# david-cortes/poismf

Hardware: AMD Instinct MI355X
Metric: nonzeros/sec per full A+B sweep (higher is better)
Workload: dtype f32; 1 GPU; uniform 1000000x100000, 99949803 nnz (100000000 triplets, seed 1, duplicates summed), k=50, method=pg, maxupd=10, l2=1000, step=1e-09

## Files before the change

poismf_amd/csrc/poismf_hip.hip:

```cpp
#include <hip/hip_runtime.h>

#include <algorithm>
#include <atomic>
#include <cstdio>
#include <cstdlib>
#include <type_traits>

#include "plan.hpp"
#include "reg_eval.hpp"
#include "lane_eval.hpp"
#include "solvers.hpp"

#ifndef PMF_TU
#define PMF_TU -1
#endif
constexpr bool tu_has(int kmethod) { return PMF_TU == -1 || PMF_TU == kmethod; }

template <class EV, class = void> struct cold_constants : std::false_type {};
template <class EV> struct cold_constants<EV, std::void_t<decltype(EV::COLD_CONSTANTS)>> : std::integral_constant<bool, EV::COLD_CONSTANTS> {};

template <class EV, class T, int NC, int METHOD>
__device__ __forceinline__ void solve_row(const HalfArgs<T>& a, EV& ev, const T (&bs)[NC], unsigned lrow, unsigned nnz)
{
    const int k = a.geom.k;
    T* out = a.M + (size_t)(a.row_offset + lrow) * (size_t)k;
    T* out_p = a.Mp != nullptr ? a.Mp + (size_t)(a.row_offset + lrow) * (size_t)a.ldM : nullptr;
    T x[NC];
    if (nnz == 0) {
        T z = (T)0;
        asm volatile("" : "+v"(z));
        PMF_EW x[i] = z;
        ev.store_vec(out, x);
        if (out_p != nullptr) ev.store_vec(out_p, x);
        return;
    }
    ev.start_point(out, x);
    ev.n_eval = 0;

    T shift[NC];
    PMF_EW shift[i] = bs[i];
    const bool weighted = a.P.w != (T)1;
    if (weighted) {
        T cs[NC];
        PMF_EW cs[i] = (T)0;
        ev.tile_colsum(cs);
        T w_here = a.P.w;
        asm volatile("" : "+v"(w_here));
        const T wm1 = w_here - (T)1.;
        PMF_EW {
            shift[i] = cs[i] * wm1;
            shift[i] = shift[i] + bs[i];
        }
        if (METHOD == K_PG) {
            PMF_EW shift[i] = shift[i] * a.P.neg_step;
            if (a.P.neg_step2 != (T)1) { PMF_EW shift[i] = shift[i] * a.P.neg_step2; }
        }
    }

    SolveStats st;
    if constexpr (METHOD == K_EVAL) {
        T g[NC];
        double f;
        if (a.P.maxupd == 0) {
            f = (double)fun_single(ev, a.P, shift, x);
            grad_single(ev, a.P, shift, x, g, weighted);
        } else f = (double)fun_and_grad(ev, a.P, shift, x, g);
        ev.store_vec(out, g);
        if (out_p != nullptr) ev.store_vec(out_p, g);
        if (a.dec_rows != nullptr && ev.lane == 0 && ev.wid == 0 && ev.member == 0) {
            const unsigned long long fb = __builtin_bit_cast(unsigned long long, f);
            a.dec_rows[2 * (size_t)lrow] = (unsigned)fb;
            a.dec_rows[2 * (size_t)lrow + 1] = (unsigned)(fb >> 32);
        }
        return;
    } else if constexpr (METHOD == K_PG) {
        pg_row(ev, a.P, x, shift);
    } else if constexpr (METHOD == K_CG) {
        if constexpr (EV::MAY_CACHE) {
            if (a.P.limit_step && ev.pq_cap > 0 && nnz <= (unsigned)ev.pq_cap) cg_row_cached(ev, a.P, shift, x, weighted, st);
            else cg_row(ev, a.P, shift, x, weighted, st);
        } else cg_row(ev, a.P, shift, x, weighted, st);
    } else {
        T prev[NC];
        PMF_EW prev[i] = x[i];
        if (!a.reuse_prev) { PMF_EW x[i] = (T)1e-3; }
        (void)Tnc<T, NC, EV>::minimize(ev, a.P, shift, x, st);
        if (a.early_stop) {
            PMF_EW prev[i] = prev[i] - x[i];
            const T moved = ev.dot(prev, prev);
            if ((double)moved <= 1e-4 && ev.lane == 0 && ev.wid == 0 && ev.member == 0) atomicAdd(a.n_unchanged, 1u);
        }
    }
    ev.store_vec(out, x);
    if (out_p != nullptr) ev.store_vec(out_p, x);
#ifndef PMF_PROBE
    if (a.eval_rows != nullptr && ev.lane == 0 && ev.wid == 0 && ev.member == 0) a.eval_rows[lrow] += ev.n_eval;
#endif
    if (a.dec_rows != nullptr && ev.lane == 0 && ev.wid == 0 && ev.member == 0) {
        unsigned d0 = (unsigned)st.niter | ((unsigned)st.rc << 24), d1 = (unsigned)st.nfeval;
        if constexpr (cold_constants<EV>::value) asm volatile("" : "+v"(d0), "+v"(d1));
        a.dec_rows[2 * (size_t)lrow] = d0;
        a.dec_rows[2 * (size_t)lrow + 1] = d1;
    }
}

template <int METHOD, class T> __device__ __forceinline__ unsigned take_ticket(const HalfArgs<T>& a)
{
    unsigned st = 0u;
    if constexpr (METHOD != K_PG) {
        if (a.stop != nullptr) st = __hip_atomic_load(a.stop, __ATOMIC_RELAXED, __HIP_MEMORY_SCOPE_SYSTEM);
    }
    const unsigned t = atomicAdd(a.queue, 1u);
    return st != 0u ? 0xffffffffu : t;
}

template <class EV, class T, int NC, int METHOD, int NW>
__device__ __forceinline__ void sweep_rows(const HalfArgs<T>& a, EV& ev, unsigned char* smem)
{
    if (a.gate != nullptr && __hip_atomic_load(a.gate, __ATOMIC_RELAXED, __HIP_MEMORY_SCOPE_AGENT) == 0) return;
    ev.init(a.geom, a.F, smem);
    T bs[NC];
    ev.load_vec(a.bsum, bs);
    const RowDesc* desc = a.desc + a.perm_begin;
    if constexpr (EV::PIPELINED && (EV::PIPE_MW == 1 || (EV::PIPE_MW == 2 && METHOD == K_PG))) {
        unsigned r = blockIdx.x;
        auto ticket = [&]() -> unsigned {
            if (a.queue != nullptr) {
                if constexpr (NW > 1) {
                    unsigned* slot = ev.ticket_slot();
                    if (threadIdx.x == 0) *slot = take_ticket<METHOD>(a);
                    __syncthreads();
                    const unsigned t = uniform(*slot);
                    __syncthreads();
                    return t;
                }
                unsigned t = 0;
                if (ev.lane == 0) t = take_ticket<METHOD>(a);
                return uniform(t);
            }
            unsigned t = r;
            r += gridDim.x;
            if constexpr (METHOD != K_PG) {
                if (a.stop != nullptr && __hip_atomic_load(a.stop, __ATOMIC_RELAXED, __HIP_MEMORY_SCOPE_SYSTEM) != 0u) t = 0xffffffffu;
            }
            return t;
        };
        auto fetch = [&](unsigned t) -> RowDesc { return desc[t < a.nrows ? t : 0u]; };
        unsigned t0 = ticket(), t1 = ticket();
        RowDesc d0 = fetch(t0), d1 = fetch(t1);
        if (t0 < a.nrows) ev.fetch_meta(a.indices + (((unsigned long long)d0.p0_hi << 32) | d0.p0_lo), d0.nnz);
#ifdef PMF_PROBE
        unsigned probe_i = 0;
#endif
        while (t0 < a.nrows) {
            const unsigned long long p0 = ((unsigned long long)d0.p0_hi << 32) | d0.p0_lo;
            if (d0.nnz != 0) ev.gather(a.values + p0, d0.nnz);
            const unsigned t2 = ticket();
            const RowDesc d2 = fetch(t2);
            if (t1 < a.nrows) ev.fetch_meta(a.indices + (((unsigned long long)d1.p0_hi << 32) | d1.p0_lo), d1.nnz);
#ifdef PMF_PROBE
            ev.probe = (a.eval_rows != nullptr && blockIdx.x == 5 && threadIdx.x < WAVE && probe_i < 60) ? a.eval_rows + 16 * probe_i : nullptr;
            if (ev.probe != nullptr && ev.lane == 0) { ev.probe[10] = (unsigned)__builtin_amdgcn_s_memtime(); ev.probe[11] = d0.nnz; }
            probe_i++;
#endif
            solve_row<EV, T, NC, METHOD>(a, ev, bs, d0.lrow, d0.nnz);
            t0 = t1; d0 = d1;
            t1 = t2; d1 = d2;
        }
        return;
    } else {
        unsigned r = blockIdx.x;
        for (;;) {
            if (a.queue != nullptr) {
                if constexpr (NW > 1) {
                    unsigned* next_row = ev.ticket_slot();
                    if (threadIdx.x == 0) *next_row = take_ticket<METHOD>(a);
                    __syncthreads();
                    r = uniform(*next_row);
                    __syncthreads();
                } else {
                    unsigned t = 0;
                    if (ev.lane == 0) t = take_ticket<METHOD>(a);
                    r = uniform(t);
                }
            }
            if (r >= a.nrows) break;
            if constexpr (METHOD != K_PG) {
                if (a.queue == nullptr && a.stop != nullptr && uniform(__hip_atomic_load(a.stop, __ATOMIC_RELAXED, __HIP_MEMORY_SCOPE_SYSTEM)) != 0u) break;
            }
            const RowDesc d = desc[r];
            r += gridDim.x;
            const unsigned nnz = uniform(d.nnz);
            const unsigned long long p0 = ((unsigned long long)uniform(d.p0_hi) << 32) | uniform(d.p0_lo);
            if (nnz != 0) ev.begin_row(a.indices + p0, a.values + p0, nnz);
            solve_row<EV, T, NC, METHOD>(a, ev, bs, uniform(d.lrow), nnz);
        }
    }
}

template <class T, int NC, int METHOD, int SL, int NW>
__global__ __launch_bounds__(WAVE* NW) void half_sweep_kernel(const HalfArgs<T> a)
{
    extern __shared__ __attribute__((aligned(16))) unsigned char smem[];
    constexpr bool PF = SL > 0 && METHOD != K_TNCG;
    RowEval<T, NC, SL, NW, PF> ev;
    if constexpr (NW > 1) {
        if (a.arrive != nullptr && threadIdx.x == 0) atomicAdd(a.arrive, 1u);
    }
#ifdef PMF_TIMING
    const unsigned long long t_kernel = __builtin_amdgcn_s_memtime();
#endif
    sweep_rows<RowEval<T, NC, SL, NW, PF>, T, NC, METHOD, NW>(a, ev, smem);
#ifdef PMF_TIMING
    ev.tacc[5] = __builtin_amdgcn_s_memtime() - t_kernel;
    if (ev.lane == 0 && ev.wid == 0)
        for (int q = 0; q < 6; q++) atomicAdd(&g_pmf_timing[q], ev.tacc[q]);
#endif
}

template <class EV, class T, int NC, int METHOD>
__device__ __forceinline__ void team_rows(const HalfArgs<T>& a, EV& ev, unsigned char* smem)
{
    if (a.arrive != nullptr && threadIdx.x == 0) atomicAdd(a.arrive, 1u);
    ev.init(a.geom, a.F, smem);
    T bs[NC];
    ev.load_vec(a.bsum, bs);
    const RowDesc* desc = a.desc + a.perm_begin;
    const unsigned M = a.team_members;
    unsigned* box = ev.ticket_slot();
    if (threadIdx.x == 0) {
        const unsigned n = atomicAdd((unsigned*)a.team_buf, 1u);
        box[0] = n / M;
        box[1] = n % M;
    }
    __syncthreads();
    const unsigned team = uniform(box[0]);
    ev.member = (int)uniform(box[1]);
    __syncthreads();
    if ((size_t)(team + 1) * gt_team_words(M) + GT_HEAD_WORDS > GT_BUF_BYTES / 8) return;
    ev.tm_M = (int)M;
    ev.tm_seq = 0;
    ev.tm_words = a.team_buf + GT_HEAD_WORDS + (size_t)team * gt_team_words(M);
    ev.tm_err = a.team_err;
    ev.tm_spin = a.team_spin;
    unsigned long long* mail = ev.tm_words;
    constexpr unsigned END = 0xffffffffu;
    if (threadIdx.x == 0) atomicAdd((unsigned*)(mail + 2), 1u);
    if (a.team_spin <= 1u && threadIdx.x == 0) __hip_atomic_store(a.team_err, 1u, __ATOMIC_RELAXED, __HIP_MEMORY_SCOPE_AGENT);
    if (ev.wid == 0) {
        for (unsigned spins = 0;; spins++) {
            if (a.team_spin <= 1u) break;
            if (uniform((unsigned)gt_load(mail + 2)) >= M) break;
            if ((spins & 255u) == 255u) {
                if (uniform(__hip_atomic_load(a.team_err, __ATOMIC_RELAXED, __HIP_MEMORY_SCOPE_AGENT)) != 0) break;
                if (uniform(__hip_atomic_load(a.queue, __ATOMIC_RELAXED, __HIP_MEMORY_SCOPE_AGENT)) >= a.nrows) break;
            }
            if ((spins >> 6) > a.team_spin) { __hip_atomic_store(a.team_err, 1u, __ATOMIC_RELAXED, __HIP_MEMORY_SCOPE_AGENT); break; }
            __builtin_amdgcn_s_sleep(8);
        }
    }
    __syncthreads();
    for (unsigned rowno = 1;; rowno++) {
        if (ev.wid == 0) {
            unsigned tk = END;
            if (ev.member == 0) {
                unsigned t0 = 0;
                if (ev.lane == 0) t0 = take_ticket<METHOD>(a);
                tk = uniform(t0);
                if (tk >= a.nrows || uniform(__hip_atomic_load(a.team_err, __ATOMIC_RELAXED, __HIP_MEMORY_SCOPE_AGENT)) != 0) tk = END;
                gt_store(mail + (rowno & 1u), ((unsigned long long)rowno << 32) | tk);
            } else {
                unsigned seen = uniform(__hip_atomic_load(a.queue, __ATOMIC_RELAXED, __HIP_MEMORY_SCOPE_AGENT));
                for (unsigned spins = 0;; spins++) {
                    const unsigned long long v = gt_load(mail + (rowno & 1u));
                    const unsigned hi = uniform((unsigned)(v >> 32)), lo = uniform((unsigned)v);
                    if (hi == rowno) { tk = lo; break; }
                    if ((spins & 255u) == 255u) {
                        if (uniform(__hip_atomic_load(a.team_err, __ATOMIC_RELAXED, __HIP_MEMORY_SCOPE_AGENT)) != 0) break;
                        const unsigned q = uniform(__hip_atomic_load(a.queue, __ATOMIC_RELAXED, __HIP_MEMORY_SCOPE_AGENT));
                        if (q != seen) { seen = q; spins = 0; }
                        else if (rowno == 1u && q >= a.nrows) break;
                    }
                    if (spins > a.team_spin) { __hip_atomic_store(a.team_err, 1u, __ATOMIC_RELAXED, __HIP_MEMORY_SCOPE_AGENT); break; }
                    __builtin_amdgcn_s_sleep(4);
                }
            }
            box[0] = tk;
        }
        __syncthreads();
        const unsigned t = uniform(box[0]);
        __syncthreads();
        if (t >= a.nrows) break;
        const RowDesc d = desc[t];
        const unsigned nnz = uniform(d.nnz);
        const unsigned long long p0 = ((unsigned long long)uniform(d.p0_hi) << 32) | uniform(d.p0_lo);
        const unsigned S = ((nnz + M - 1u) / M + (EV::TEAM_ROUND - 1u)) / EV::TEAM_ROUND * EV::TEAM_ROUND;
        const unsigned off = (unsigned)ev.member * S;
        const unsigned mine = off < nnz ? (nnz - off < S ? nnz - off : S) : 0u;
        ev.begin_row(a.indices + p0 + (mine ? off : 0u), a.values + p0 + (mine ? off : 0u), mine);
        solve_row<EV, T, NC, METHOD>(a, ev, bs, uniform(d.lrow), nnz);
    }
}
template <class T, int NC, int METHOD, int SL, int NW>
__global__ __launch_bounds__(WAVE* NW) void half_sweep_giant_kernel(const HalfArgs<T> a)
{
    extern __shared__ __attribute__((aligned(16))) unsigned char smem[];
    constexpr bool PF = SL > 0 && METHOD != K_TNCG;
    using EV = RowEval<T, NC, SL, NW, PF, true>;
    EV ev;
// ... 542 lines not shown
```

poismf_amd/csrc/reg_eval.hpp:

```cpp
#pragma once
#include <type_traits>

#include "row_eval.hpp"

namespace pmf {

template <int I, int N, class Fn> __device__ __forceinline__ void static_for(Fn&& f)
{
    if constexpr (I < N) {
        f(std::integral_constant<int, I>{});
        static_for<I + 1, N>(f);
    }
}

template <int G, int U> __device__ __forceinline__ int group_bcast_i32(int v)
{
    return __builtin_amdgcn_ds_swizzle(v, (0x1f & ~(G - 1)) | (U << 5));
}
template <int G, int U> __device__ __forceinline__ unsigned group_bcast(unsigned v) { return (unsigned)group_bcast_i32<G, U>((int)v); }
template <int G, int U> __device__ __forceinline__ float group_bcast(float v)
{
    return __builtin_bit_cast(float, group_bcast_i32<G, U>(__builtin_bit_cast(int, v)));
}
template <int G, int U> __device__ __forceinline__ double group_bcast(double v)
{
    if constexpr (G == 16) return __builtin_amdgcn_update_dpp(0.0, v, 0x150 + U, 0xf, 0xf, true);
    const unsigned long long b = __builtin_bit_cast(unsigned long long, v);
    const unsigned lo = (unsigned)group_bcast_i32<G, U>((int)(unsigned)b);
    const unsigned hi = (unsigned)group_bcast_i32<G, U>((int)(unsigned)(b >> 32));
    return __builtin_bit_cast(double, ((unsigned long long)hi << 32) | lo);
}

template <int CTRL, class T> __device__ __forceinline__ T fold_pair(bool cls, T pa, T pb)
{
    const T own = cls ? pb : pa;
    const T send = cls ? pa : pb;
    return own + dpp_mov<CTRL>(send);
}
template <int CTRL, class T> __device__ __forceinline__ T fold_one(T pa) { return pa + dpp_mov<CTRL>(pa); }

template <int CTRL, int H, int NIN, class T> __device__ __forceinline__ void fold_level(bool cls, const T* in, T* out)
{
#pragma unroll
    for (int i = 0; i < H; i++) {
        if (i + H < NIN) out[i] = fold_pair<CTRL>(cls, in[i], in[i + H]);
        else if (i < NIN) out[i] = fold_one<CTRL>(in[i]);
        else out[i] = (T)0;
    }
}

__device__ __forceinline__ float coef_div(float num, float den)
{
    const float r = __builtin_amdgcn_rcpf(den);
    float q = num * r;
    const float e = __builtin_fmaf(-den, q, num);
    q = __builtin_fmaf(e, r, q);
    return __builtin_amdgcn_div_fixupf(q, den, num);
}
__device__ __forceinline__ double coef_div(double num, double den) { return num / den; }

#define PMF_FOLD2(CTRL, M0, M1, Q, A, B) \
    "v_add_f32_dpp " Q ", " A ", " A " " CTRL " row_mask:0xf bank_mask:" M0 "\n\t" \
    "v_add_f32_dpp " Q ", " B ", " B " " CTRL " row_mask:0xf bank_mask:" M1 "\n\t"
__device__ __forceinline__ void fold16_banked(const float (&p)[16], float (&q)[8])
{
    asm("s_nop 1\n\t"
        PMF_FOLD2("row_ror:8", "0x3", "0xc", "%0", "%8", "%16")
        PMF_FOLD2("row_ror:8", "0x3", "0xc", "%1", "%9", "%17")
        PMF_FOLD2("row_ror:8", "0x3", "0xc", "%2", "%10", "%18")
        PMF_FOLD2("row_ror:8", "0x3", "0xc", "%3", "%11", "%19")
        PMF_FOLD2("row_ror:8", "0x3", "0xc", "%4", "%12", "%20")
        PMF_FOLD2("row_ror:8", "0x3", "0xc", "%5", "%13", "%21")
        PMF_FOLD2("row_ror:8", "0x3", "0xc", "%6", "%14", "%22")
        PMF_FOLD2("row_ror:8", "0x3", "0xc", "%7", "%15", "%23")
        : "=&v"(q[0]), "=&v"(q[1]), "=&v"(q[2]), "=&v"(q[3]), "=&v"(q[4]), "=&v"(q[5]), "=&v"(q[6]), "=&v"(q[7])
        : "v"(p[0]), "v"(p[1]), "v"(p[2]), "v"(p[3]), "v"(p[4]), "v"(p[5]), "v"(p[6]), "v"(p[7]),
          "v"(p[8]), "v"(p[9]), "v"(p[10]), "v"(p[11]), "v"(p[12]), "v"(p[13]), "v"(p[14]), "v"(p[15]));
}
__device__ __forceinline__ void fold8_banked(const float (&q)[8], float (&r)[4])
{
    asm("s_nop 1\n\t"
        PMF_FOLD2("row_half_mirror", "0x5", "0xa", "%0", "%4", "%8")
        PMF_FOLD2("row_half_mirror", "0x5", "0xa", "%1", "%5", "%9")
        PMF_FOLD2("row_half_mirror", "0x5", "0xa", "%2", "%6", "%10")
        PMF_FOLD2("row_half_mirror", "0x5", "0xa", "%3", "%7", "%11")
        : "=&v"(r[0]), "=&v"(r[1]), "=&v"(r[2]), "=&v"(r[3])
        : "v"(q[0]), "v"(q[1]), "v"(q[2]), "v"(q[3]), "v"(q[4]), "v"(q[5]), "v"(q[6]), "v"(q[7]));
}

__device__ __forceinline__ void gran_store(unsigned long long* p, unsigned long long v)
{
    __hip_atomic_store(p, v, __ATOMIC_RELAXED, __HIP_MEMORY_SCOPE_AGENT);
}
__device__ __forceinline__ unsigned long long gran_load(const unsigned long long* p)
{
    return __hip_atomic_load(p, __ATOMIC_RELAXED, __HIP_MEMORY_SCOPE_AGENT);
}

template <class T, int S, int G_ = 16, int NS_ = 1, int NW_ = 1, int M_ = 1, bool PAIR_ = false> struct RegEval {
    using SA = typename Slot<T>::A;
    using SU = typename Slot<T>::U;
    static constexpr int SN = Slot<T>::N;
    static constexpr int G = G_, NS = NS_;
    static constexpr bool PAIRED = PAIR_;
    static_assert(!PAIR_ || (SN == 4 && G_ == 16 && NS_ == 1 && NW_ == 1 && M_ == 1 && S % 2 == 0), "step pairs: fp32 one-wave tiles of whole pairs");
    typedef T V2 __attribute__((ext_vector_type(2)));
    static constexpr int JG = WAVE / G;
    static constexpr int NC = NS * SN;
    static constexpr int NB = (S + G - 1) / G;
    static constexpr int NW = NW_;
    static constexpr bool PIPELINED = true;
    static constexpr int PIPE_MW = 1;
    static constexpr bool FUSED_SUMS = false;
    static constexpr bool PREFETCH = false;
    static constexpr int KP = G * NS * SN;
    static constexpr int M = M_;
    static constexpr int RED_BYTES = NW_ * KP * (int)sizeof(T) + (M_ > 1 ? NW_ * 8 * TEAM_SC : 16 * ((NW_ * 8 + 15) / 16));
    static constexpr int TEAM_BYTES = M_ > 1 ? KP * (int)sizeof(T) + 8 * TEAM_SC : 0;
    static constexpr bool PARKS = sizeof(T) == 8 && M_ > 1;
    static constexpr int PARK_SLOTS = 6;
    static constexpr int PARK_BYTES = PARKS ? NW_ * PARK_SLOTS * KP * (int)sizeof(T) : 0;
    static constexpr int PARK_OFFSET = (NW_ > 1 ? 2 * RED_BYTES + 16 : 0) + TEAM_BYTES;
    static constexpr int SMEM_BYTES = PARK_OFFSET + PARK_BYTES;
    static_assert(M_ == 1 || (sizeof(T) == 8 && NW_ > 1 && NS_ * Slot<T>::N <= WAVE / G_), "teams: doubles, one element per group to publish");
    static_assert(G == 8 || G == 16, "a factor row is held by 8 or 16 lanes");

    SA t[PAIRED ? 1 : S][NS];
    V2 tp[PAIRED ? S / 2 : 1][SN];
    T a[NC];
    T xr[NB];
    unsigned idx_n[NB];
    const T* F;
    unsigned zero_row;
    int k, ldF, s_load;
    int lane, g, jg, wid;
    int jlane;
    bool cls8, cls4, cls2, cls1;
    struct ElemOf {
        int g;
        __device__ __forceinline__ int operator[](int i) const { return (g + G * (i / SN)) * SN + i % SN; }
    } elem;
    bool act[NC];
    bool slot_on[NS];
    unsigned nnz;
    unsigned n_eval;
#ifdef PMF_PROBE
    unsigned* probe = nullptr;
    unsigned long long probe_wait = 0;
    unsigned long long probe_acc[8] = {0, 0, 0, 0, 0, 0, 0, 0};
#endif
    unsigned char* red_base;
    int red_sel;
    unsigned* ticket_word;
    T* park_base;
    unsigned long long* team_words;
    unsigned* team_err;
    unsigned team_spin = TEAM_SPIN_LIMIT;
    T* team_tot;
    int member;
    unsigned xseq;
    int pq_cap;
    T* pbuf;
    T* qbuf;
    static constexpr bool CACHED = (sizeof(T) == 8 && (NW_ == 1 || M_ > 1)) || sizeof(T) == 4;
    static constexpr bool MAY_CACHE = CACHED;
    static constexpr bool CACHED_GRAD = CACHED;
    T pv[CACHED ? NB : 1], qv[CACHED ? NB : 1];

    __device__ __forceinline__ void init(const TileGeom& geo, const T* F_, unsigned char* smem)
    {
        lane = lane_id();
        red_base = smem;
        red_sel = 0;
        ticket_word = (unsigned*)(smem + 2 * RED_BYTES);
        team_tot = (T*)(smem + 2 * RED_BYTES + 16);
        park_base = (T*)(smem + PARK_OFFSET) + (NW > 1 ? (int)(threadIdx.x / WAVE) : 0) * PARK_SLOTS * KP;
        member = 0; xseq = 0; team_words = nullptr; team_err = nullptr;
        F = F_;
        k = geo.k; ldF = geo.ldF; s_load = geo.s_load; zero_row = geo.zero_row;
        g = lane & (G - 1); elem.g = g; jg = lane / G; wid = NW > 1 ? (int)(threadIdx.x / WAVE) : 0;
        jlane = JG * g + jg;
        cls8 = (lane & 8) != 0; cls4 = (lane & 4) != 0; cls2 = (lane & 2) != 0; cls1 = (lane & 1) != 0;
#pragma unroll
        for (int n = 0; n < NS; n++) {
            const int q = g + G * n;
            slot_on[n] = q < s_load;
#pragma unroll
            for (int e = 0; e < SN; e++) {
                act[n * SN + e] = q * SN + e < k;
            }
        }
        pq_cap = CACHED ? 0x7fffffff : 0;
        pbuf = (T*)(size_t)16; qbuf = (T*)(size_t)32;
    }

    template <class Op, class V> __device__ __forceinline__ V reduce(V x) const
    {
        x = Op::f(x, dpp_mov<0xB1>(x));
        x = Op::f(x, dpp_mov<0x4E>(x));
        x = Op::f(x, dpp_mov<0x141>(x));
        if constexpr (G == 16) x = Op::f(x, dpp_mov<0x140>(x));
        return uniform(x);
    }
    template <class V> __device__ __forceinline__ V rsum(V x) const { return reduce<OpSum>(x); }
    template <class V> __device__ __forceinline__ V rmin(V x) const { return reduce<OpMin>(x); }
    template <class V> __device__ __forceinline__ V rmax(V x) const { return reduce<OpMax>(x); }
    __device__ __forceinline__ T dot(const T (&u)[NC], const T (&v)[NC]) const
    {
        T s = (T)0;
#pragma unroll
        for (int i = 0; i < NC; i++) s = act[i] ? fma_t(u[i], v[i], s) : s;
        return rsum(s);
    }
    __device__ __forceinline__ T nrm2(const T (&u)[NC]) const { return (T)d_sqrt((double)dot(u, u)); }
    __device__ __forceinline__ void start_point(const T* mrow, T (&x)[NC]) const { load_vec(mrow, x); }
    __device__ __forceinline__ void load_vec(const T* p, T (&x)[NC]) const
    {
#pragma unroll
        for (int n = 0; n < NS; n++) {
            SU v;
#pragma unroll
            for (int e = 0; e < SN; e++) v.v[e] = (T)0;
            if (slot_on[n]) v = *(const SU*)(p + (g + G * n) * SN);
#pragma unroll
            for (int e = 0; e < SN; e++) x[n * SN + e] = act[n * SN + e] ? v.v[e] : (T)0;
        }
    }
    __device__ __forceinline__ void store_vec(T* p, const T (&x)[NC]) const
    {
        if (jg == 0 && wid == 0 && member == 0) {
#pragma unroll
            for (int n = 0; n < NS; n++) {
                if (act[n * SN + SN - 1]) {
                    SU v;
#pragma unroll
                    for (int e = 0; e < SN; e++) v.v[e] = x[n * SN + e];
                    *(SU*)(p + (g + G * n) * SN) = v;
                } else {
#pragma unroll
                    for (int e = 0; e < SN; e++)
                        if (act[n * SN + e]) p[elem[n * SN + e]] = x[n * SN + e];
                }
            }
        }
    }

    __device__ __forceinline__ void park(int slot, const T (&x)[NC])
    {
        if (jg == 0) {
#pragma unroll
            for (int n = 0; n < NS; n++) {
                SA v;
#pragma unroll
                for (int e = 0; e < SN; e++) v.v[e] = x[n * SN + e];
                *(SA*)(park_base + slot * KP + (g + G * n) * SN) = v;
            }
        }
    }
    __device__ __forceinline__ void unpark(int slot, T (&x)[NC])
    {
#ifdef PMF_PROBE
        const unsigned long long t_up0 = __builtin_amdgcn_s_memtime();
        struct UpTimer { unsigned long long& acc; unsigned long long t0; __device__ ~UpTimer() { acc += __builtin_amdgcn_s_memtime() - t0; } } up_timer{ probe_acc[3], t_up0 };
#endif
        wave_lds_fence();
#pragma unroll
        for (int n = 0; n < NS; n++) {
            const SA v = *(const SA*)(park_base + slot * KP + (g + G * n) * SN);
#pragma unroll
            for (int e = 0; e < SN; e++) x[n * SN + e] = v.v[e];
        }
    }

    __device__ __forceinline__ void my_share(unsigned nnz_row, unsigned& c0, unsigned& mine) const
    {
        if constexpr (NW > 1) {
            const unsigned C = ((nnz_row + NW * M - 1) / (NW * M) + JG - 1) / JG * JG;
            c0 = (unsigned)(member * NW + wid) * C;
            mine = c0 < nnz_row ? (nnz_row - c0 < C ? nnz_row - c0 : C) : 0u;
        } else {
            c0 = 0u; mine = nnz_row;
        }
    }
    __device__ __forceinline__ void fetch_meta(const unsigned* ind, unsigned nnz_row)
    {
        unsigned c0, mine;
        my_share(nnz_row, c0, mine);
#pragma unroll
        for (int b = 0; b < NB; b++) {
            const unsigned j = (unsigned)(64 * b + jlane);
            idx_n[b] = j < mine ? ind[c0 + j] : zero_row;
        }
    }
    __device__ __forceinline__ void begin_row(const unsigned* ind, const T* val, unsigned nnz_row)
    {
        fetch_meta(ind, nnz_row);
        gather(val, nnz_row);
    }
    __device__ __forceinline__ unsigned* ticket_slot() const { return ticket_word; }

    __device__ __forceinline__ void team_exchange(T (&tot)[NC], double (&sc)[TEAM_SC], bool vec)
    {
        if constexpr (M > 1) {
            xseq++;
            double* team_l = (double*)(team_tot + KP);
            if (wid == 0) {
                const unsigned long long tag = (unsigned long long)xseq << 32;
                unsigned long long* slots = team_words + 2 + TEAM_M_MAX + (size_t)(xseq & 1u) * TEAM_M_MAX * TEAM_GRAN;
                const bool carrier = vec && jg < NC;
                const bool scalar = lane < TEAM_SC;
                T mine = tot[0];
#pragma unroll
                for (int i = 1; i < NC; i++) { mine = jg == i ? tot[i] : mine; asm volatile("" : "+v"(mine)); }
                double mysc = sc[0];
#pragma unroll
                for (int j = 1; j < TEAM_SC; j++) { mysc = lane == j ? sc[j] : mysc; asm volatile("" : "+v"(mysc)); }
                if (carrier) {
                    const unsigned long long b = __builtin_bit_cast(unsigned long long, (double)mine);
                    gran_store(slots + member * TEAM_GRAN + 2 * lane, (b & 0xffffffffull) | tag);
                    gran_store(slots + member * TEAM_GRAN + 2 * lane + 1, (b >> 32) | tag);
                }
                if (scalar) {
                    const unsigned long long b = __builtin_bit_cast(unsigned long long, mysc);
                    gran_store(slots + member * TEAM_GRAN + 128 + 2 * lane, (b & 0xffffffffull) | tag);
                    gran_store(slots + member * TEAM_GRAN + 129 + 2 * lane, (b >> 32) | tag);
                }
                T sum = (T)0;
                double lt = 0.0;
#pragma unroll
                for (int m = 0; m < M; m++) {
                    T pv = mine;
                    double pl = mysc;
                    if (m != member) {
#ifdef PMF_PROBE
                        const unsigned long long t_wait0 = __builtin_amdgcn_s_memtime();
// ... 2 lines not shown
                        unsigned long long a0 = tag, a1 = tag, l0 = tag, l1 = tag;
                        unsigned spins = 0;
                        for (;;) {
                            if (carrier) { a0 = gran_load(theirs + 2 * lane); a1 = gran_load(theirs + 2 * lane + 1); }
                            if (scalar) { l0 = gran_load(theirs + 128 + 2 * lane); l1 = gran_load(theirs + 129 + 2 * lane); }
                            const bool ok = (a0 >> 32) == xseq && (a1 >> 32) == xseq && (l0 >> 32) == xseq && (l1 >> 32) == xseq;
                            if (__builtin_amdgcn_ballot_w64(!ok) == 0) break;
                            __builtin_amdgcn_s_sleep(1);
                            if ((++spins & 255u) == 0 && (spins > team_spin || __hip_atomic_load(team_err, __ATOMIC_RELAXED, __HIP_MEMORY_SCOPE_AGENT) != 0)) {
                                if (lane == 0) __hip_atomic_store(team_err, 1u, __ATOMIC_RELAXED, __HIP_MEMORY_SCOPE_AGENT);
                                break;
                            }
                        }
                        pv = (T)__builtin_bit_cast(double, (a0 & 0xffffffffull) | (a1 << 32));
                        pl = __builtin_bit_cast(double, (l0 & 0xffffffffull) | (l1 << 32));
#ifdef PMF_PROBE
                        probe_wait += __builtin_amdgcn_s_memtime() - t_wait0;
#endif
                    }
                    sum = m == 0 ? pv : sum + pv;
                    lt = m == 0 ? pl : lt + pl;
                }
                if (carrier) team_tot[elem[jg < NC ? jg : 0]] = sum;
                if (scalar) team_l[lane] = lt;
            }
            __syncthreads();
            if (vec) {
#pragma unroll
                for (int n = 0; n < NS; n++) {
                    const SA v = *(const SA*)(team_tot + (g + G * n) * SN);
#pragma unroll
                    for (int e = 0; e < SN; e++) tot[n * SN + e] = act[n * SN + e] ? v.v[e] : (T)0;
                }
            }
#pragma unroll
            for (int j = 0; j < TEAM_SC; j++) sc[j] = team_l[j];
        }
    }
    __device__ __forceinline__ void combine_scalars(double (&sc)[TEAM_SC])
    {
        if constexpr (M > 1) {
            double* red_l = (double*)(red_base + red_sel * RED_BYTES + NW * KP * sizeof(T));
            red_sel ^= 1;
            double mysc = sc[0];
#pragma unroll
            for (int j = 1; j < TEAM_SC; j++) { mysc = lane == j ? sc[j] : mysc; asm volatile("" : "+v"(mysc)); }
            if (lane < TEAM_SC) red_l[wid * TEAM_SC + lane] = mysc;
            __syncthreads();
#pragma unroll
            for (int j = 0; j < TEAM_SC; j++) {
                double t = 0.0;
#pragma unroll
                for (int w = 0; w < NW; w++) t += red_l[w * TEAM_SC + j];
                sc[j] = t;
            }
            T none[NC];
#pragma unroll
            for (int i = 0; i < NC; i++) none[i] = (T)0;
            team_exchange(none, sc, false);
        }
    }

    __device__ __forceinline__ void combine_waves(T (&tot)[NC], double& lsum, bool vec = true)
    {
        if constexpr (NW > 1) {
            T* red_part = (T*)(red_base + red_sel * RED_BYTES);
            double* red_l = (double*)(red_base + red_sel * RED_BYTES + NW * KP * sizeof(T));
            red_sel ^= 1;
            SA* red_slots = (SA*)red_part;
            if (jg == 0 && (M == 1 || vec)) {
#pragma unroll
                for (int n = 0; n < NS; n++) {
                    SA v;
#pragma unroll
                    for (int e = 0; e < SN; e++) v.v[e] = tot[n * SN + e];
                    red_slots[wid * (G * NS) + g + G * n] = v;
                }
            }
            if (lane == 0) red_l[wid] = lsum;
            __syncthreads();
            PMF_STAMP(*this, 7);
            if constexpr (NW <= 8) {
                double lp[NW];
#pragma unroll
                for (int w = 0; w < NW; w++) lp[w] = red_l[w];
                lsum = 0.0;
#pragma unroll
                for (int w = 0; w < NW; w++) lsum += lp[w];
                if (M == 1 || vec) {
                    SA part[NW][NS];
#pragma unroll
                    for (int w = 0; w < NW; w++) {
#pragma unroll
                        for (int n = 0; n < NS; n++) part[w][n] = red_slots[w * (G * NS) + g + G * n];
                    }
#pragma unroll
                    for (int i = 0; i < NC; i++) tot[i] = (T)0;
#pragma unroll
                    for (int w = 0; w < NW; w++) {
#pragma unroll
                        for (int n = 0; n < NS; n++) {
#pragma unroll
                            for (int e = 0; e < SN; e++) tot[n * SN + e] += act[n * SN + e] ? part[w][n].v[e] : (T)0;
                        }
                    }
                }
                if constexpr (M > 1) {
                    double sc[TEAM_SC];
#pragma unroll
                    for (int j = 0; j < TEAM_SC; j++) sc[j] = 0.0;
                    sc[0] = lsum;
                    team_exchange(tot, sc, vec);
                    lsum = sc[0];
                }
            } else {
                lsum = 0.0;
#pragma unroll
                for (int i = 0; i < NC; i++) tot[i] = (T)0;
#pragma unroll
                for (int w0 = 0; w0 < NW; w0 += 8) {
                    SA part[8][NS];
                    double lp[8];
#pragma unroll
                    for (int w = 0; w < 8; w++) {
                        lp[w] = red_l[w0 + w];
#pragma unroll
                        for (int n = 0; n < NS; n++) part[w][n] = red_slots[(w0 + w) * (G * NS) + g + G * n];
                    }
#pragma unroll
                    for (int w = 0; w < 8; w++) {
                        lsum += lp[w];
#pragma unroll
                        for (int n = 0; n < NS; n++) {
#pragma unroll
                            for (int e = 0; e < SN; e++) tot[n * SN + e] += act[n * SN + e] ? part[w][n].v[e] : (T)0;
                        }
                    }
                }
            }
        }
    }
    __device__ __forceinline__ void gather(const T* val, unsigned nnz_row)
    {
        unsigned c0;
        my_share(nnz_row, c0, nnz);
        unsigned idx[NB];
#pragma unroll
        for (int b = 0; b < NB; b++) {
            const unsigned j = (unsigned)(64 * b + jlane);
            idx[b] = idx_n[b];
            xr[b] = j < nnz ? val[c0 + j] : (T)0;
        }
        const unsigned rowbytes = (unsigned)ldF * (unsigned)sizeof(T);
        unsigned lane_off[NS];
#pragma unroll
        for (int n = 0; n < NS; n++) lane_off[n] = slot_on[n] ? (unsigned)((g + G * n) * 16) : 0u;
        SU raw[PAIRED ? S : 1];
        static_for<0, S>([&](auto sc) {
            constexpr int s = decltype(sc)::value;
            const unsigned c = group_bcast<G, s % G>(idx[s / G]);
#pragma unroll
            for (int n = 0; n < NS; n++) {
                const unsigned off = __umul24(slot_on[n] ? c : zero_row, rowbytes) + lane_off[n];
                const SU v = *(const SU*)((const char*)F + (size_t)off);
                if constexpr (PAIRED) raw[s] = v;
                else {
#pragma unroll
                    for (int e = 0; e < SN; e++) t[s][n].v[e] = v.v[e];
                }
            }
        });
        if constexpr (PAIRED) {
#pragma unroll
            for (int i = 0; i < S / 2; i++) {
                T x1 = raw[2 * i].v[1], y0 = raw[2 * i + 1].v[0], x3 = raw[2 * i].v[3], y2 = raw[2 * i + 1].v[2];
                asm("v_swap_b32 %0, %1\n\tv_swap_b32 %2, %3" : "+v"(x1), "+v"(y0), "+v"(x3), "+v"(y2));
                tp[i][0] = (V2){ raw[2 * i].v[0], x1 };
                tp[i][1] = (V2){ y0, raw[2 * i + 1].v[1] };
                tp[i][2] = (V2){ raw[2 * i].v[2], x3 };
                tp[i][3] = (V2){ y2, raw[2 * i + 1].v[3] };
            }
        }
    }
    __device__ __forceinline__ void set_point(const T (&x)[NC])
    {
#pragma unroll
        for (int i = 0; i < NC; i++) a[i] = act[i] ? x[i] : (T)0;
    }

    __device__ __forceinline__ T lane_dot(const SA (&w)[NS]) const
    {
        if constexpr (SN == 4) {
            typedef T V2 __attribute__((ext_vector_type(2)));
            V2 p = (V2){ w[0].v[0], w[0].v[1] } * (V2){ a[0], a[1] };
            p = __builtin_elementwise_fma((V2){ w[0].v[2], w[0].v[3] }, (V2){ a[2], a[3] }, p);
#pragma unroll
            for (int n = 1; n < NS; n++) {
                p = __builtin_elementwise_fma((V2){ w[n].v[0], w[n].v[1] }, (V2){ a[4 * n], a[4 * n + 1] }, p);
                p = __builtin_elementwise_fma((V2){ w[n].v[2], w[n].v[3] }, (V2){ a[4 * n + 2], a[4 * n + 3] }, p);
            }
            return p.x + p.y;
        } else {
            T p = fma_t(w[0].v[1], a[1], w[0].v[0] * a[0]);
#pragma unroll
            for (int n = 1; n < NS; n++) {
                p = fma_t(w[n].v[0], a[2 * n], p);
                p = fma_t(w[n].v[1], a[2 * n + 1], p);
            }
            return p;
        }
    }

    __device__ __forceinline__ V2 lane_dot2(const V2 (&w)[SN]) const
    {
        V2 p = w[0] * (V2){ a[0], a[0] };
#pragma unroll
        for (int e = 1; e < SN; e++) p = __builtin_elementwise_fma(w[e], (V2){ a[e], a[e] }, p);
        return p;
    }
    __device__ __forceinline__ T tile_at(int s, int m, int e) const
    {
        if constexpr (PAIRED) return tp[s / 2][e][s % 2];
        else return t[s][m].v[e];
    }

    template <int N> __device__ __forceinline__ T transpose_sum(const T (&p)[G]) const
    {
        T q[8], r[4], s2[2];
        constexpr int N8 = N < 8 ? N : 8;
        constexpr bool F32 = std::is_same<T, float>::value;
        if constexpr (F32 && G == 16 && N == 16) fold16_banked(p, q);
        else if constexpr (G == 16) fold_level<0x128, 8, N>(cls8, p, q);
        else {
#pragma unroll
            for (int i = 0; i < 8; i++) q[i] = p[i];
        }
        if constexpr (F32 && N8 == 8) fold8_banked(q, r);
        else fold_level<0x141, 4, N8>(cls4, q, r);
        constexpr int N4 = N8 < 4 ? N8 : 4;
        fold_level<0x4E, 2, N4>(cls2, r, s2);
        constexpr int N2 = N4 < 2 ? N4 : 2;
        if constexpr (N2 == 2) return fold_pair<0xB1>(cls1, s2[0], s2[1]);
        else return fold_one<0xB1>(s2[0]);
    }

    __device__ __forceinline__ void combine_groups(T (&part)[NC], T (&acc)[NC]) const
    {
        if constexpr (G == 8) {
#pragma unroll
            for (int i = 0; i < NC; i++) part[i] += dpp_mov<0x128>(part[i]);
        }
        if constexpr (sizeof(T) == 8) {
#pragma unroll
            for (int i = 0; i < NC; i++) part[i] = xor_sum<16>(part[i]);
#pragma unroll
            for (int i = 0; i < NC; i++) part[i] = xor_sum<32>(part[i]);
        } else {
#pragma unroll
            for (int i = 0; i < NC; i++) part[i] += __shfl_xor(part[i], 16);
#pragma unroll
            for (int i = 0; i < NC; i++) part[i] += __shfl_xor(part[i], 32);
        }
#pragma unroll
        for (int i = 0; i < NC; i++) acc[i] += part[i];
    }

    template <bool WANT_F, bool WANT_G, bool FROM_CACHE = false> __device__ __forceinline__ double eval(T sgn, T (&acc)[NC], T* store = nullptr)
    {
        n_eval++;
        PMF_STAMP(*this, 0);
#ifdef PMF_PROBE
        const unsigned long long t_eval0 = __builtin_amdgcn_s_memtime();
        struct EvalTimer { unsigned long long& acc; unsigned long long t0; __device__ ~EvalTimer() { acc += __builtin_amdgcn_s_memtime() - t0; } } eval_timer{ probe_acc[0], t_eval0 };
#endif
        double lpart = 0.0;
        T part[NC];
#pragma unroll
        for (int i = 0; i < NC; i++) part[i] = (T)0;
        V2 part2[PAIRED ? SN : 1];
#pragma unroll
        for (int i = 0; i < (PAIRED ? SN : 1); i++) part2[i] = (V2){ (T)0, (T)0 };
        static_for<0, NB>([&](auto bc) {
            constexpr int b = decltype(bc)::value;
            constexpr int n = (S - G * b) < G ? (S - G * b) : G;
            T pred;
            if constexpr (FROM_CACHE && CACHED) pred = pv[b];
            else {
                T p[G];
                if constexpr (PAIRED) {
#pragma unroll
                    for (int i = 0; i < G / 2; i++) {
                        const V2 q = 2 * i < n ? lane_dot2(tp[(G * b + 2 * i) < S ? (G * b) / 2 + i : 0]) : (V2){ (T)0, (T)0 };
                        p[2 * i] = q.x;
                        p[2 * i + 1] = q.y;
                    }
                } else {
#pragma unroll
                    for (int u = 0; u < G; u++) p[u] = u < n ? lane_dot(t[(G * b + u) < S ? (G * b + u) : 0]) : (T)0;
                }
                if constexpr (b == 0) PMF_STAMP(*this, 1);
                pred = transpose_sum<n>(p);
                if constexpr (b == 0) PMF_STAMP(*this, 2);
            }
            if constexpr (CACHED) {
                if (store == pbuf) pv[b] = pred;
                else if (store == qbuf) qv[b] = pred;
            }
            const bool on = (unsigned)(64 * b + jlane) < nnz;
            const T xj = xr[b];
            if constexpr (WANT_F) lpart += on ? (double)xj * d_log((double)pred) : 0.0;
            if constexpr (WANT_G) {
                const T coef = on ? coef_div(sgn * xj, pred) : (T)0;
                if constexpr (b == 0) PMF_STAMP(*this, 3);
                if constexpr (PAIRED) {
                    static_for<0, n / 2>([&](auto ic) {
                        constexpr int i = decltype(ic)::value;
                        const V2 c = { group_bcast<G, 2 * i>(coef), group_bcast<G, 2 * i + 1>(coef) };
#pragma unroll
                        for (int e = 0; e < SN; e++) part2[e] = __builtin_elementwise_fma(c, tp[(G * b) / 2 + i][e], part2[e]);
                    });
                } else {
                    static_for<0, n>([&](auto uc) {
                        constexpr int u = decltype(uc)::value;
                        const T c = group_bcast<G, u>(coef);
#pragma unroll
                        for (int m = 0; m < NS; m++) {
#pragma unroll
                            for (int e = 0; e < SN; e++) part[m * SN + e] = fma_t(c, t[G * b + u][m].v[e], part[m * SN + e]);
                        }
                    });
                }
                if constexpr (b == 0) PMF_STAMP(*this, 4);
            }
        });
        if constexpr (PAIRED && WANT_G) {
#pragma unroll
            for (int e = 0; e < SN; e++) asm("v_add_f32 %0, %1, %2" : "=v"(part[e]) : "v"(part2[e].x), "v"(part2[e].y));
        }
        PMF_STAMP(*this, 5);
        if constexpr (NW > 1 && !WANT_F && !WANT_G) {
            return 0.0;
        } else if constexpr (NW > 1) {
            T tot[NC];
#pragma unroll
            for (int i = 0; i < NC; i++) tot[i] = (T)0;
            if constexpr (WANT_G) combine_groups(part, tot);
            PMF_STAMP(*this, 6);
            double lsum = 0.0;
            if constexpr (WANT_F) lsum = wave_sum(lpart);
#ifdef PMF_PROBE
            const unsigned long long t_cw0 = __builtin_amdgcn_s_memtime();
#endif
            combine_waves(tot, lsum, WANT_G);
#ifdef PMF_PROBE
            probe_acc[1] += __builtin_amdgcn_s_memtime() - t_cw0;
#endif
            PMF_STAMP(*this, 8);
            if constexpr (WANT_G) {
#pragma unroll
                for (int i = 0; i < NC; i++) acc[i] += tot[i];
            }
            return lsum;
        } else {
            if constexpr (WANT_G) combine_groups(part, acc);
            PMF_STAMP(*this, 6);
            if constexpr (WANT_F) return wave_sum(lpart);
            else return 0.0;
        }
    }

    __device__ __forceinline__ double logsum_cached(T alpha, bool& trusted)
    {
        double lpart = 0.0;
        bool bad = false;
#pragma unroll
        for (int b = 0; b < (CACHED ? NB : 0); b++) {
            const bool on = (unsigned)(64 * b + jlane) < nnz;
            const T pred = fma_t(alpha, qv[b], pv[b]);
            bad = bad || (on && !(pred > pv[b] * (T)1e-4));
            lpart += on ? (double)xr[b] * d_log((double)pred) : 0.0;
        }
        trusted = __builtin_amdgcn_ballot_w64(bad) == 0;
        double l = wave_sum(lpart);
        if constexpr (NW > 1) {
            if (!trusted) l = __builtin_nan("");
            T none[NC];
#pragma unroll
            for (int i = 0; i < NC; i++) none[i] = (T)0;
            combine_waves(none, l, false);
            trusted = !(l != l);
        }
        return l;
    }
#ifndef PMF_TEAM_LSB
#define PMF_TEAM_LSB 4
#endif
    static constexpr int LS_BATCH = M_ > 1 ? PMF_TEAM_LSB : 1;
    __device__ __forceinline__ void logsum_cached_batch(T alpha, T decr, double (&ls)[LS_BATCH], bool (&trusted)[LS_BATCH])
    {
        if constexpr (M > 1) {
#ifdef PMF_PROBE
            const unsigned long long t_ls0 = __builtin_amdgcn_s_memtime();
            struct LsTimer { unsigned long long& acc; unsigned long long t0; __device__ ~LsTimer() { acc += __builtin_amdgcn_s_memtime() - t0; } } ls_timer{ probe_acc[2], t_ls0 };
#endif
            T al = alpha;
#pragma unroll
            for (int j = 0; j < LS_BATCH; j++) {
                double lpart = 0.0;
                bool bad = false;
#pragma unroll
                for (int b = 0; b < (CACHED ? NB : 0); b++) {
                    const bool on = (unsigned)(64 * b + jlane) < nnz;
                    const T pred = fma_t(al, qv[b], pv[b]);
                    bad = bad || (on && !(pred > pv[b] * (T)1e-4));
                    lpart += on ? (double)xr[b] * d_log((double)pred) : 0.0;
                }
                const double l = wave_sum(lpart);
                ls[j] = __builtin_amdgcn_ballot_w64(bad) == 0 ? l : __builtin_nan("");
                al *= decr;
            }
            double sc[TEAM_SC];
#pragma unroll
            for (int j = 0; j < TEAM_SC; j++) sc[j] = j < LS_BATCH ? ls[j < LS_BATCH ? j : 0] : 0.0;
#ifdef PMF_PROBE
            const unsigned long long t_cs0 = __builtin_amdgcn_s_memtime();
#endif
            combine_scalars(sc);
#ifdef PMF_PROBE
            probe_acc[7] += __builtin_amdgcn_s_memtime() - t_cs0;
#endif
#pragma unroll
            for (int j = 0; j < LS_BATCH; j++) { ls[j] = sc[j]; trusted[j] = !(ls[j] != ls[j]); }
        } else {
            ls[0] = logsum_cached(alpha, trusted[0]);
        }
    }
    __device__ __forceinline__ void advance_cached(T alpha)
    {
#pragma unroll
        for (int b = 0; b < (CACHED ? NB : 0); b++) pv[b] = fma_t(alpha, qv[b], pv[b]);
    }

#ifdef PMF_PROBE
    __device__ __forceinline__ void tile_touch(T (&acc)[NC])
    {
#pragma unroll
        for (int s = 0; s < S; s++) acc[0] += tile_at(s, 0, 0) + tile_at(s, NS - 1, SN - 1);
    }
#endif
    __device__ __forceinline__ void tile_colsum(T (&acc)[NC])
    {
        T part[NC];
#pragma unroll
        for (int i = 0; i < NC; i++) part[i] = (T)0;
#pragma unroll
        for (int s = 0; s < S; s++) {
#pragma unroll
            for (int m = 0; m < NS; m++) {
#pragma unroll
                for (int e = 0; e < SN; e++) part[m * SN + e] += tile_at(s, m, e);
            }
        }
        if constexpr (NW > 1) {
            T tot[NC];
#pragma unroll
            for (int i = 0; i < NC; i++) tot[i] = (T)0;
            combine_groups(part, tot);
            double unused = 0.0;
            combine_waves(tot, unused);
#pragma unroll
            for (int i = 0; i < NC; i++) acc[i] += tot[i];
        } else {
            combine_groups(part, acc);
        }
    }
};

}
```

poismf_amd/csrc/solvers.hpp:

```cpp
#pragma once
#include <type_traits>
#include <utility>

#include "row_eval.hpp"

namespace pmf {

#define PMF_EW _Pragma("unroll") for (int i = 0; i < NC; i++)

template <class T> __device__ __forceinline__ bool not_finite(T v) { return isnan(v) || isinf(v); }

struct SolveStats { int niter = 0, nfeval = 0, rc = 0; };

template <class EV, class T, int NC>
__device__ __forceinline__ void pg_row(EV& ev, const RowParams<T>& P, T (&x)[NC], const T (&shift)[NC])
{
    for (int u = 0; u < P.maxupd; u++) {
        ev.set_point(x);
        T g[NC];
        PMF_EW g[i] = (T)0;
        ev.template eval<false, true>((T)1, g);
        PMF_EW {
            x[i] = fma_t(P.step, g[i], x[i]);
            x[i] = x[i] + shift[i];
            x[i] = x[i] * P.cnst_div;
            x[i] = (x[i] > (T)0) ? x[i] : (T)0;
        }
        PMF_STAMP(ev, 9);
    }
}

template <class EV, class T, int NC>
__device__ __forceinline__ T fun_single(EV& ev, const RowParams<T>& P, const T (&bsum)[NC], const T (&a)[NC])
{
    ev.set_point(a);
    T dummy[NC];
    PMF_EW dummy[i] = (T)0;
    T reg = ev.dot(bsum, a);
    reg += P.l2 * ev.dot(a, a);
    const T lsum = (T)ev.template eval<true, false>((T)0, dummy);
    return reg - lsum * P.w;
}

template <class EV, class T, int NC>
__device__ __forceinline__ void grad_single(EV& ev, const RowParams<T>& P, const T (&bsum)[NC],
                                            const T (&a)[NC], T (&g)[NC], bool weighted)
{
    ev.set_point(a);
    const T two_l2 = (T)(2. * (double)P.l2);
    if (!weighted) {
        PMF_EW g[i] = fma_t(two_l2, a[i], bsum[i]);
        ev.template eval<false, true>((T)-1, g);
    } else {
        PMF_EW g[i] = (T)0;
        ev.template eval<false, true>((T)-1, g);
        PMF_EW {
            g[i] = g[i] * P.w;
            g[i] = g[i] + bsum[i];
            g[i] = fma_t(two_l2, a[i], g[i]);
        }
    }
}

template <class EV, class T, int NC>
__device__ __forceinline__ T fun_and_grad(EV& ev, const RowParams<T>& P, const T (&bsum)[NC],
                                          const T (&a)[NC], T (&g)[NC])
{
    ev.set_point(a);
#ifdef PMF_DUP_EVAL
    {
        T g2[NC];
        PMF_EW g2[i] = (T)0;
        const double l2nd = ev.template eval<true, true>((T)-1, g2);
        asm volatile("" :: "v"(g2[0]), "v"(l2nd));
        ev.n_eval--;
    }
#endif
    PMF_EW g[i] = (T)0;
    const T lsum = (T)ev.template eval<true, true>((T)-1, g);
    const T two_l2 = (T)(2. * (double)P.l2);
    if (P.w != (T)1) { PMF_EW g[i] = g[i] * P.w; }
    PMF_EW g[i] = g[i] + bsum[i];
    const T reg = ev.dot(bsum, a);
    PMF_EW g[i] = fma_t(two_l2, a[i], g[i]);
    return reg - lsum * P.w;
}

template <class T>
__device__ __forceinline__ bool skip_certain_failures(T f_x, T f_cur, T gd, T l2dd, T dd, T c_ls, T decr, int max_ls, int maxnfeval,
                                                      T& step, int& ls, int& nfeval)
{
    const T eps_m = sizeof(T) == 8 ? (T)1e-9 : (T)1e-3;
    const T marg = eps_m * (T)(d_abs((double)f_x) + d_abs((double)f_cur));
    while (ls < max_ls - 1) {
        const T lb = fma_t(step * step, l2dd, fma_t(step, gd, f_x));
        const T thr = f_cur - c_ls * step * dd;
        if (!(lb > thr + marg)) break;
        nfeval++;
        if (nfeval >= maxnfeval) return false;
        step *= decr;
        ls++;
    }
    return true;
}

template <class EV, class T, int NC>
__device__ __forceinline__ void cg_row(EV& ev, const RowParams<T>& P, const T (&bsum)[NC], T (&x)[NC],
                                       bool weighted, SolveStats& st)
{
    const T tol = (T)1e-2, decr = (T)0.25, c_ls = (T)0.01;
    const int maxnfeval = 150, max_ls = 20;
    const int maxiter = P.maxupd > 0 ? P.maxupd : 0x7fffffff;
    T g[NC], d[NC], gp[NC], dp[NC], trial[NC];
    PMF_EW { gp[i] = (T)0; dp[i] = (T)0; }
    T gprev_sq = (T)0;
    T f_cur = fun_single(ev, P, bsum, x);
    T f_new = (T)0;
    T f_x = f_cur;
    int nfeval = 1;
    int it = 0;
    auto leave = [&](int rc) { st.niter = it; st.nfeval = nfeval; st.rc = rc; };
    if (not_finite(f_cur)) { leave(3); return; }
    const bool prune = P.x_pos != 0 && P.limit_step != 0;

    for (it = 0; it < maxiter; it++) {
        grad_single(ev, P, bsum, x, g, weighted);
        PMF_EW d[i] = (x[i] <= (T)0 && g[i] >= (T)0) ? (T)0 : -g[i];
        if (it > 0) {
            T th = (T)0, be = (T)0;
            PMF_EW {
                const bool on = ev.act[i] && !(x[i] <= (T)0);
                th += on ? g[i] * dp[i] : (T)0;
                be += on ? g[i] * (g[i] - gp[i]) : (T)0;
            }
            T theta = ev.rsum(th), beta = ev.rsum(be);
            theta /= gprev_sq;
            beta /= gprev_sq;
            PMF_EW d[i] += (x[i] <= (T)0) ? (T)0 : beta * dp[i] - theta * (g[i] - gp[i]);
        }
        const T gd = ev.dot(g, d);
        if (d_abs((double)gd) <= (double)tol) { leave(0); return; }

        T max_step;
        if (P.limit_step) {
            T m = (T)1;
            PMF_EW if (ev.act[i] && d[i] < (T)0) m = (T)d_min((double)m, (double)(-x[i] / d[i]));
            max_step = ev.rmin(m);
        } else {
            T m = (T)0;
            PMF_EW if (ev.act[i] && d[i] < (T)0) m = (T)d_max((double)m, (double)(-x[i] / d[i]));
            max_step = ev.rmax(m);
            max_step = (T)d_min(1., 0.99 * (double)max_step);
        }

        const T dd = ev.dot(d, d);
        T step = max_step;
        int ls = 0;
        if (prune && !skip_certain_failures(f_x, f_cur, gd, P.l2 * dd, dd, c_ls, decr, max_ls, maxnfeval, step, ls, nfeval)) { leave(1); return; }
        for (; ls < max_ls; ls++) {
            PMF_EW {
                trial[i] = fma_t(step, d[i], x[i]);
                if (P.limit_step) trial[i] = ((double)trial[i] >= 1e-15) ? trial[i] : (T)0;
                else              trial[i] = (trial[i] > (T)0) ? trial[i] : (T)0;
            }
            f_new = fun_single(ev, P, bsum, trial);
            if (!not_finite(f_new) && f_new <= f_cur - c_ls * step * dd) {
                PMF_EW x[i] = trial[i];
                f_x = f_new;
                break;
            }
            nfeval++;
            if (nfeval >= maxnfeval) { leave(1); return; }
            step *= decr;
        }
// ... 828 lines not shown
```

Measured before the change: 10.96 billion nnz/s.

## Trim PG inner loop: lean set_point, fresh gradient accumulate, cheaper cross-lane reductions

Adds several micro-optimizations to the register evaluator. It precomputes the per-lane row multiplier and offset, so inactive slots read a zero row without a per-element select in the gather. It replaces the xor-16/32 shuffles with a ds_swizzle and a ds_bpermute that uses a precomputed address, and adds a 12-wide banked DPP fold. For the PG method it skips the active-mask select in set_point and writes the gradient directly instead of accumulating into zeros. Idle tiles with zero nonzeros clear the paired tile registers. The ROOMY choice trades register pressure against the gather path depending on tile size, which risks spills for some configurations.

```diff
diff --git a/poismf_amd/csrc/poismf_hip.hip b/poismf_amd/csrc/poismf_hip.hip
--- a/poismf_amd/csrc/poismf_hip.hip
+++ b/poismf_amd/csrc/poismf_hip.hip
@@ -18,6 +18,9 @@
 
 template <class EV, class = void> struct cold_constants : std::false_type {};
 template <class EV> struct cold_constants<EV, std::void_t<decltype(EV::COLD_CONSTANTS)>> : std::integral_constant<bool, EV::COLD_CONSTANTS> {};
+
+template <class EV, class = void> struct has_idle_tile : std::false_type {};
+template <class EV> struct has_idle_tile<EV, std::void_t<decltype(&EV::idle_tile)>> : std::true_type {};
 
 template <class EV, class T, int NC, int METHOD>
 __device__ __forceinline__ void solve_row(const HalfArgs<T>& a, EV& ev, const T (&bs)[NC], unsigned lrow, unsigned nnz)
@@ -155,6 +158,7 @@
         while (t0 < a.nrows) {
             const unsigned long long p0 = ((unsigned long long)d0.p0_hi << 32) | d0.p0_lo;
             if (d0.nnz != 0) ev.gather(a.values + p0, d0.nnz);
+            else if constexpr (has_idle_tile<EV>::value) ev.idle_tile();
             const unsigned t2 = ticket();
             const RowDesc d2 = fetch(t2);
             if (t1 < a.nrows) ev.fetch_meta(a.indices + (((unsigned long long)d1.p0_hi << 32) | d1.p0_lo), d1.nnz);
diff --git a/poismf_amd/csrc/reg_eval.hpp b/poismf_amd/csrc/reg_eval.hpp
--- a/poismf_amd/csrc/reg_eval.hpp
+++ b/poismf_amd/csrc/reg_eval.hpp
@@ -77,6 +77,22 @@
         : "v"(p[0]), "v"(p[1]), "v"(p[2]), "v"(p[3]), "v"(p[4]), "v"(p[5]), "v"(p[6]), "v"(p[7]),
           "v"(p[8]), "v"(p[9]), "v"(p[10]), "v"(p[11]), "v"(p[12]), "v"(p[13]), "v"(p[14]), "v"(p[15]));
 }
+#define PMF_FOLD1(CTRL, Q, A) "v_add_f32_dpp " Q ", " A ", " A " " CTRL " row_mask:0xf bank_mask:0xf\n\t"
+__device__ __forceinline__ void fold12_banked(const float (&p)[16], float (&q)[8])
+{
+    asm("s_nop 1\n\t"
+        PMF_FOLD2("row_ror:8", "0x3", "0xc", "%0", "%8", "%16")
+        PMF_FOLD2("row_ror:8", "0x3", "0xc", "%1", "%9", "%17")
+        PMF_FOLD2("row_ror:8", "0x3", "0xc", "%2", "%10", "%18")
+        PMF_FOLD2("row_ror:8", "0x3", "0xc", "%3", "%11", "%19")
+        PMF_FOLD1("row_ror:8", "%4", "%12")
+        PMF_FOLD1("row_ror:8", "%5", "%13")
+        PMF_FOLD1("row_ror:8", "%6", "%14")
+        PMF_FOLD1("row_ror:8", "%7", "%15")
+        : "=&v"(q[0]), "=&v"(q[1]), "=&v"(q[2]), "=&v"(q[3]), "=&v"(q[4]), "=&v"(q[5]), "=&v"(q[6]), "=&v"(q[7])
+        : "v"(p[0]), "v"(p[1]), "v"(p[2]), "v"(p[3]), "v"(p[4]), "v"(p[5]), "v"(p[6]), "v"(p[7]),
+          "v"(p[8]), "v"(p[9]), "v"(p[10]), "v"(p[11]));
+}
 __device__ __forceinline__ void fold8_banked(const float (&q)[8], float (&r)[4])
 {
     asm("s_nop 1\n\t"
@@ -103,6 +119,7 @@
     static constexpr int SN = Slot<T>::N;
     static constexpr int G = G_, NS = NS_;
     static constexpr bool PAIRED = PAIR_;
+    static constexpr bool ROOMY = !(PAIR_ && S >= 40);
     static_assert(!PAIR_ || (SN == 4 && G_ == 16 && NS_ == 1 && NW_ == 1 && M_ == 1 && S % 2 == 0), "step pairs: fp32 one-wave tiles of whole pairs");
     typedef T V2 __attribute__((ext_vector_type(2)));
     static constexpr int JG = WAVE / G;
@@ -136,6 +153,7 @@
     int lane, g, jg, wid;
     int jlane;
     bool cls8, cls4, cls2, cls1;
+    int xor32_addr;
     struct ElemOf {
         int g;
         __device__ __forceinline__ int operator[](int i) const { return (g + G * (i / SN)) * SN + i % SN; }
@@ -181,6 +199,8 @@
         g = lane & (G - 1); elem.g = g; jg = lane / G; wid = NW > 1 ? (int)(threadIdx.x / WAVE) : 0;
         jlane = JG * g + jg;
         cls8 = (lane & 8) != 0; cls4 = (lane & 4) != 0; cls2 = (lane & 2) != 0; cls1 = (lane & 1) != 0;
+        xor32_addr = (lane ^ 32) << 2;
+        asm volatile("" : "+v"(xor32_addr));
 #pragma unroll
         for (int n = 0; n < NS; n++) {
             const int q = g + G * n;
@@ -489,16 +509,27 @@
             xr[b] = j < nnz ? val[c0 + j] : (T)0;
         }
         const unsigned rowbytes = (unsigned)ldF * (unsigned)sizeof(T);
-        unsigned lane_off[NS];
-#pragma unroll
-        for (int n = 0; n < NS; n++) lane_off[n] = slot_on[n] ? (unsigned)((g + G * n) * 16) : 0u;
+        unsigned lane_mul[NS], lane_off[NS];
+#pragma unroll
+        for (int n = 0; n < NS; n++) {
+            const unsigned slot_off = (unsigned)((g + G * n) * 16);
+            if constexpr (ROOMY) {
+                lane_mul[n] = slot_on[n] ? rowbytes : 0u;
+                lane_off[n] = slot_on[n] ? slot_off : __umul24(zero_row, rowbytes);
+            } else {
+                lane_mul[n] = rowbytes;
+                lane_off[n] = slot_on[n] ? slot_off : 0u;
+            }
+        }
         SU raw[PAIRED ? S : 1];
         static_for<0, S>([&](auto sc) {
             constexpr int s = decltype(sc)::value;
             const unsigned c = group_bcast<G, s % G>(idx[s / G]);
 #pragma unroll
             for (int n = 0; n < NS; n++) {
-                const unsigned off = __umul24(slot_on[n] ? c : zero_row, rowbytes) + lane_off[n];
+                unsigned row = c;
+                if constexpr (!ROOMY) row = slot_on[n] ? c : zero_row;
+                const unsigned off = __umul24(row, lane_mul[n]) + lane_off[n];
                 const SU v = *(const SU*)((const char*)F + (size_t)off);
                 if constexpr (PAIRED) raw[s] = v;
                 else {
@@ -519,10 +550,28 @@
             }
         }
     }
+    __device__ __forceinline__ void idle_tile()
+    {
+        if constexpr (PAIRED) {
+            asm volatile("" ::: "memory");
+#pragma unroll
+            for (int i = 0; i < S / 2; i++) {
+#pragma unroll
+                for (int e = 0; e < SN; e++) tp[i][e] = (V2){ (T)0, (T)0 };
+            }
+        }
+    }
     __device__ __forceinline__ void set_point(const T (&x)[NC])
     {
 #pragma unroll
         for (int i = 0; i < NC; i++) a[i] = act[i] ? x[i] : (T)0;
+    }
+
+    static constexpr bool PG_LEAN = ROOMY;
+    __device__ __forceinline__ void set_point_as_is(const T (&x)[NC])
+    {
+#pragma unroll
+        for (int i = 0; i < NC; i++) a[i] = x[i];
     }
 
     __device__ __forceinline__ T lane_dot(const SA (&w)[NS]) const
@@ -567,6 +616,7 @@
         constexpr int N8 = N < 8 ? N : 8;
         constexpr bool F32 = std::is_same<T, float>::value;
         if constexpr (F32 && G == 16 && N == 16) fold16_banked(p, q);
+        else if constexpr (F32 && G == 16 && N == 12) fold12_banked(p, q);
         else if constexpr (G == 16) fold_level<0x128, 8, N>(cls8, p, q);
         else {
 #pragma unroll
@@ -581,7 +631,7 @@
         else return fold_one<0xB1>(s2[0]);
     }
 
-    __device__ __forceinline__ void combine_groups(T (&part)[NC], T (&acc)[NC]) const
+    template <bool FRESH = false> __device__ __forceinline__ void combine_groups(T (&part)[NC], T (&acc)[NC]) const
     {
         if constexpr (G == 8) {
 #pragma unroll
@@ -594,15 +644,15 @@
             for (int i = 0; i < NC; i++) part[i] = xor_sum<32>(part[i]);
         } else {
 #pragma unroll
-            for (int i = 0; i < NC; i++) part[i] += __shfl_xor(part[i], 16);
-#pragma unroll
-            for (int i = 0; i < NC; i++) part[i] += __shfl_xor(part[i], 32);
-        }
-#pragma unroll
-        for (int i = 0; i < NC; i++) acc[i] += part[i];
-    }
-
-    template <bool WANT_F, bool WANT_G, bool FROM_CACHE = false> __device__ __forceinline__ double eval(T sgn, T (&acc)[NC], T* store = nullptr)
+            for (int i = 0; i < NC; i++) part[i] += __builtin_bit_cast(T, __builtin_amdgcn_ds_swizzle(__builtin_bit_cast(int, part[i]), 0x401f));
+#pragma unroll
+            for (int i = 0; i < NC; i++) part[i] += __builtin_bit_cast(T, __builtin_amdgcn_ds_bpermute(xor32_addr, __builtin_bit_cast(int, part[i])));
+        }
+#pragma unroll
+        for (int i = 0; i < NC; i++) acc[i] = FRESH ? part[i] : acc[i] + part[i];
+    }
+
+    template <bool WANT_F, bool WANT_G, bool FROM_CACHE = false, bool FRESH = false> __device__ __forceinline__ double eval(T sgn, T (&acc)[NC], T* store = nullptr)
     {
         n_eval++;
         PMF_STAMP(*this, 0);
@@ -681,7 +731,7 @@
             T tot[NC];
 #pragma unroll
             for (int i = 0; i < NC; i++) tot[i] = (T)0;
-            if constexpr (WANT_G) combine_groups(part, tot);
+            if constexpr (WANT_G) combine_groups<true>(part, tot);
             PMF_STAMP(*this, 6);
             double lsum = 0.0;
             if constexpr (WANT_F) lsum = wave_sum(lpart);
@@ -695,11 +745,11 @@
             PMF_STAMP(*this, 8);
             if constexpr (WANT_G) {
 #pragma unroll
-                for (int i = 0; i < NC; i++) acc[i] += tot[i];
+                for (int i = 0; i < NC; i++) acc[i] = FRESH ? tot[i] : acc[i] + tot[i];
             }
             return lsum;
         } else {
-            if constexpr (WANT_G) combine_groups(part, acc);
+            if constexpr (WANT_G) combine_groups<FRESH>(part, acc);
             PMF_STAMP(*this, 6);
             if constexpr (WANT_F) return wave_sum(lpart);
             else return 0.0;
diff --git a/poismf_amd/csrc/solvers.hpp b/poismf_amd/csrc/solvers.hpp
--- a/poismf_amd/csrc/solvers.hpp
+++ b/poismf_amd/csrc/solvers.hpp
@@ -11,15 +11,23 @@
 template <class T> __device__ __forceinline__ bool not_finite(T v) { return isnan(v) || isinf(v); }
 
 struct SolveStats { int niter = 0, nfeval = 0, rc = 0; };
+
+template <class EV, class = void> struct pg_lean : std::false_type {};
+template <class EV> struct pg_lean<EV, std::void_t<decltype(EV::PG_LEAN)>> : std::integral_constant<bool, EV::PG_LEAN> {};
 
 template <class EV, class T, int NC>
 __device__ __forceinline__ void pg_row(EV& ev, const RowParams<T>& P, T (&x)[NC], const T (&shift)[NC])
 {
     for (int u = 0; u < P.maxupd; u++) {
-        ev.set_point(x);
         T g[NC];
         PMF_EW g[i] = (T)0;
-        ev.template eval<false, true>((T)1, g);
+        if constexpr (pg_lean<EV>::value) {
+            ev.set_point_as_is(x);
+            ev.template eval<false, true, false, true>((T)1, g);
+        } else {
+            ev.set_point(x);
+            ev.template eval<false, true>((T)1, g);
+        }
         PMF_EW {
             x[i] = fma_t(P.step, g[i], x[i]);
             x[i] = x[i] + shift[i];
```

New measurement: 11.14 billion nnz/s, median of 6. 1.7% higher.
